# ccuchengwei/LongReadSelfCorrect

Measured on AMD Instinct MI355X. Metric: corrected Mbases/s (whole node), higher is better.
Workload: dtype int64

## Files before the change

longreadselfcorrect_amd/csrc/capi_core.cpp:

```cpp
#include <cmath>
#include <limits>

#include "capi_internal.h"

using namespace lrsc;

static thread_local std::string g_last_error;

int lrsc::fail(int status, const std::string& msg)
{
    g_last_error = msg;
    return status;
}
int lrsc::hip_fail(hipError_t e, const char* what)
{
    g_last_error = std::string(what) + ": " + hipGetErrorString(e);
    return LRSC_ERR_DEVICE;
}

extern "C" const char* lrsc_strerror(int status)
{
    switch(status) {
        case LRSC_OK: return "ok";
        case LRSC_ERR_IO: return "I/O error";
// ... 61 lines not shown
    (void)hipDeviceGetAttribute(&cus, hipDeviceAttributeMultiprocessorCount, ctx->device);
    return (uint32_t)cus * 4u * per_simd;
}

Tunables lrsc::read_tunables(const lrsc_ctx* ctx)
{
    const int kIntMax = std::numeric_limits<int>::max();
    Tunables t;
    t.wp_prep_bytes = env_bytes("LRSC_WP_PREP_MB", 24ull << 30, 20);
    t.wp_lane_bytes = env_bytes("LRSC_WP_LANE_MB", 32ull << 30, 20);
    t.wp_lanes = env_clamped("LRSC_WP_LANES", resident_waves(ctx, 2) * 64u, 64, kIntMax);
    t.wp_gen_quorum = env_clamped("LRSC_WP_GEN_QUORUM", 70, 0, 100);
    t.wp_gen_wait = env_clamped("LRSC_WP_GEN_WAIT", 6, 0, kIntMax);
    t.wp_wide_cap = env_clamped("LRSC_WP_WIDE_CAP", kNarrowLeaves, 1, (int)kNarrowLeaves);
    t.wp_wave = env_clamped("LRSC_WP_WAVE", 1, 0, 2);
    { const char* e = std::getenv("LRSC_WP_BEGIN_SORT"); t.wp_begin_sort = e && e[0] != '0'; }
    t.dp_chunk_bytes = env_bytes("LRSC_DP_CHUNK_MB", 16ull << 30, 20);
    t.dp_align_waves = env_clamped("LRSC_DP_ALIGN_WAVES", 0, 0, kIntMax);
    t.msa_force_global = std::getenv("LRSC_MSA_FORCE_GLOBAL") != nullptr;
    t.msa_lds_max = env_clamped("LRSC_MSA_LDS_MAX", 0, 1, kIntMax);
    { const char* e = std::getenv("LRSC_MSA_BATCH"); t.msa_batch = !(e && e[0] == '0'); }
    t.profile = std::getenv("LRSC_CORRECT_PROFILE") != nullptr;
    t.wp_dump = std::getenv("LRSC_WP_DUMP") != nullptr;
    t.dp_debug = std::getenv("LRSC_DP_DEBUG") != nullptr;
    return t;
}

int lrsc::check_offsets(const uint64_t* off, uint32_t n_reads)
{
    if(!off) return fail(LRSC_ERR_ARG, "null read offsets");
// ... 128 lines not shown
```

longreadselfcorrect_amd/csrc/capi_correct.cpp:

```cpp
#include "capi_internal.h"

using namespace lrsc;

struct lrsc::CorrectScratch {
    DevBuf<ReadPlan> d_plan;
    DevBuf<uint32_t> d_pieces;
    DevBuf<uint8_t> d_codes_out;
    DevBuf<uint64_t> d_dst_off;
    DevBuf<char> d_dst;
    DevBuf<double> d_freqs;
    DpStage stage;
    DevBuf<WpReadWork> d_work;
    DevBuf<WpRead> d_reads;
    DevBuf<WpSlot> d_slots;
    DevBuf<uint64_t> d_sz;
    DevBuf<uint32_t> d_key, d_key_tmp, d_list, d_list_tmp;
    DevBuf<uint32_t> d_small;
    DevBuf<WpDpItem> d_items, d_items2, d_items3;
    DevBuf<DevCounters> d_ctr2;
    hipEvent_t ev_side_t0 = nullptr, ev_side_t1 = nullptr;
    DevBuf<WpRequest> d_req;
    DevBuf<uint8_t> d_prep, d_lane, d_lane_side, d_lane_wide;
    DevBuf<uint32_t> d_wide_list;
    DevBuf<uint32_t> d_sort9;
// ... 165 lines not shown
    a.plan_stats = small(kWpSmallPlanStats); a.queue = small(kWpSmallQueue); a.n_dp_items = small(kWpSmallDpItems);
    a.n_req_out = small(kWpSmallReqOut);
    a.n_sort9 = small(kWpSmallSort9); a.begin_sort = tn.wp_begin_sort ? 1u : 0u;
    a.req_out = sc.d_req.p; a.req_cap = n;
    a.out_codes = sc.d_codes_out.p; a.piece_start = sc.d_pieces.p;
    a.auto_dp = (!p.no_dp && p.next_target == 1) ? 1u : 0u;
    a.general_quorum_pct = tn.wp_gen_quorum; a.general_max_wait = tn.wp_gen_wait;
    a.ctr = ctx->d_ctr;
    if(b->debug_flags & LRSC_DEBUG_WALKS) {
        if(!b->d_walk_log) HIP_TRY(hipMalloc(reinterpret_cast<void**>(&b->d_walk_log), b->seed_cap));
        HIP_TRY(hipMemsetAsync(b->d_walk_log, 0, b->seed_cap, ctx->stream));
        a.walk_log = b->d_walk_log;
        b->walk_log_done = false;
    }
    if(tn.profile) {
        HIP_TRY(sc.d_prof.reserve(36));
        HIP_TRY(hipMemsetAsync(sc.d_prof.p, 0, 36 * sizeof(unsigned long long), ctx->stream));
        a.prof = sc.d_prof.p;
        a.begin_stats = sc.d_prof.p + 32;
    }
    if(!sc.side) {
        int least = 0, greatest = 0;
        HIP_TRY(hipDeviceGetStreamPriorityRange(&least, &greatest));
        HIP_TRY(hipStreamCreateWithPriority(&sc.side, hipStreamNonBlocking, least));
    }
    if(!sc.ev_ready) HIP_TRY(hipEventCreateWithFlags(&sc.ev_ready, hipEventDisableTiming));
    return LRSC_OK;
}

void WpFlow::choose_range(uint32_t first)
{
    r0 = r1 = first;
// ... 127 lines not shown
    const WpLaneLayout LL = wp_lane_layout(lbytes, pathw);
    const uint64_t slots = tn.wp_lanes / 64;
    const uint64_t share = side ? wp_side_waves(tn) : slots;
    uint64_t lanes = std::min<uint64_t>(stride == 1 ? (((uint64_t)count + 63) & ~63ull) : count, share * 64 / stride);
    lanes = std::max<uint64_t>(1, std::min<uint64_t>(lanes, (tn.wp_lane_bytes / (side ? 4 : 1)) / LL.total));
    if(stride == 1) lanes = std::max<uint64_t>(64, lanes & ~63ull);
    DevBuf<uint8_t>& buf = side ? sc.d_lane_side : sc.d_lane;
    hipError_t e = buf.reserve(lanes * LL.total);
    if(e != hipSuccess) return e;
    x.list = list; x.reqs = rq; x.n_list = count;
    x.lane_ws = buf.p; x.lane_ws_bytes = LL.total; x.lane_pathw = pathw; x.n_lanes = (uint32_t)lanes; x.lane_stride = stride;
    x.queue = small(side ? kWpSmallSideQueue : kWpSmallExtQueue);
    e = hipMemsetAsync(x.queue, 0, sizeof(uint32_t), st);
    if(e != hipSuccess) return e;
    if(stride == 64 && tn.wp_wave != 0) return launch_wp_extend_wave(ctx->fm, x, st);
    return launch_wp_extend(ctx->fm, x, st);
}

int WpFlow::extension_launches(Round& R)
{
    return timed_launch(ctx, LRSC_K_EXTEND, [&]() -> hipError_t {
        hipError_t e = launch_wp_prepare(ctx->fm, a, ctx->stream);
        if(e == hipSuccess) e = launch_wp_begin(ctx->fm, a, ctx->stream);
        if(e != hipSuccess) return e;
        if(R.index != 0)
            return extend_range(a, a.list, a.reqs, R.n_ent, std::max(R.stats[2], 1u), ctx->stream, false,
                                R.n_ent <= 16384 ? 64u : R.n_ent <= 65536 ? 16u : 1u);
        e = extend_range(a, R.ext_list + R.n_mid, nullptr, R.n_ent - R.n_mid, std::min(R.stats[2], kWpPathwSmall), ctx->stream, false, 1);
        if(e != hipSuccess || R.n_mid == 0) return e;
        if(p.no_dp || escalate) return extend_range(a, R.ext_list, nullptr, R.n_mid, R.stats[2], ctx->stream, false, 64);
        R.long_launch = true;
        return e;
    });
}

int WpFlow::escalate_walks(const WpArgs& x0, uint32_t n_ent, uint32_t pathw)
{
    HIP_TRY(sc.d_wide_list.reserve(n_ent));
    uint32_t* d_count = small(kWpSmallWideCount);
    HIP_TRY(hipMemsetAsync(d_count, 0, sizeof(uint32_t), ctx->stream));
    hipError_t e = launch_wp_wide_collect(x0, sc.d_wide_list.p, d_count, ctx->stream);
    if(e != hipSuccess) return hip_fail(e, "wp_wide_collect");
    uint32_t n_wide = 0;
// ... 152 lines not shown
{
    std::fprintf(stderr, "[lrsc] wp reads [%u, %u) round %u: %u entries, %u DP requests (%llu strings), arenas q %.1f MB prep %.1f MB path %.1f MB, %llu walks escalated so far\n",
                 r0, r1, R.index, R.n_ent, R.n_items, (unsigned long long)sc.stage.n_strings, R.tot[0] / 1048576.0, R.tot[1] / 1048576.0, R.tot[2] / 1048576.0,
                 (unsigned long long)n_escalated);
    const unsigned long long* g = R.begin_stats;
    if(tn.wp_begin_sort)
        std::fprintf(stderr, "[lrsc] wp reads [%u, %u) round %u: wp_begin %llu interval lists, %llu entries, every list sorted (LRSC_WP_BEGIN_SORT)\n",
                     r0, r1, R.index, g[0], g[2] + g[3]);
    else
        std::fprintf(stderr, "[lrsc] wp reads [%u, %u) round %u: wp_begin %llu interval lists, %llu with a repeated code (%.1f%%); entries %llu in the lists without one, %llu in those with one\n",
                     r0, r1, R.index, g[0], g[1], 100.0 * g[1] / std::max(g[0], 1ull), g[2], g[3]);
}

int WpFlow::print_extension_profile()
{
    unsigned long long prs[32];
    HIP_TRY(hipStreamSynchronize(ctx->stream));
    HIP_TRY(hipStreamSynchronize(sc.side));
    HIP_TRY(hipMemcpy(prs, sc.d_prof.p, sizeof(prs), hipMemcpyDeviceToHost));
    for(int part = 0; part < 2; ++part) {
        const unsigned long long* pr = prs + 16 * part;
        if(pr[10] == 0) continue;
        const double all = (double)pr[10], st = (double)std::max<unsigned long long>(pr[11], 1);
        std::fprintf(stderr, "[lrsc] wp extension kernel (%s), lane wall ticks: %.3g total, %.0f per step over %.3g steps; extendLeaves %.1f%% (refine %.1f%%, attempToExtend %.1f%% of which "
                             "getFMIndexExtensions %.1f%%; SelectFreqsOfrange %.1f%%), PrunedBySeedSupport %.1f%%, materialise+commit %.1f%%, isTerminated %.1f%%, refill %.1f%%, finish %.1f%%; single-leaf fast steps %.1f%% of the steps in %.1f%% of the ticks\n",
                     part ? "long-gap walks, one per wavefront" : "bulk and later rounds",
                     all, all / st, st, 100 * pr[0] / all, 100 * pr[1] / all, 100 * pr[2] / all, 100 * pr[3] / all, 100 * pr[13] / all, 100 * pr[4] / all, 100 * pr[5] / all, 100 * pr[6] / all,
                     100 * pr[8] / all, 100 * pr[9] / all, 100 * pr[12] / st, 100 * pr[7] / all);
    }
    return LRSC_OK;
}

int WpFlow::gather_results(lrsc_read_result* res, uint64_t* piece_off, uint64_t piece_cap, char* out, uint64_t out_cap,
                           uint64_t* n_pieces_out, uint64_t* out_used)
{
    std::vector<WpRead> ro(n);
    COPY_TRY(ctx, ro.data(), sc.d_reads.p, (size_t)n * sizeof(WpRead), hipMemcpyDeviceToHost);
    std::vector<uint32_t> pieces(std::max<uint64_t>(piece_total, 1));
    if(piece_total) COPY_TRY(ctx, pieces.data(), sc.d_pieces.p, (size_t)piece_total * sizeof(uint32_t), hipMemcpyDeviceToHost);
    std::vector<uint64_t> dst_off(n + 1, 0);
    uint64_t n_pieces = 0;
    for(uint32_t r = 0; r < n; ++r) {
        const WpRead& o = ro[r];
// ... 81 lines not shown
```

longreadselfcorrect_amd/csrc/capi_internal.h:

```cpp
#pragma once
#include <hip/hip_runtime_api.h>

#include <algorithm>
#include <cstdint>
#include <cstdio>
#include <cstdlib>
#include <cstring>
#include <map>
#include <mutex>
#include <new>
#include <string>
#include <vector>

#include "../../include/lrsc.h"
#include "fm_layout.h"
#include "fm_locate.h"
#include "fm_pack.h"
#include "kernels.h"
#include "extend.h"
#include "correct_dev.h"
#include "dp_dev.h"
#include "wp.h"
#include "saipb.h"

// ... 43 lines not shown
            ++cur; off = 0;
        }
        auto* c = new(std::nothrow) DevBuf<uint8_t>();
        if(!c) return hipErrorOutOfMemory;
        hipError_t e = c->reserve(std::max<size_t>(bytes + bytes / 8, 64u << 20));
        if(e != hipSuccess) { delete c; return e; }
        chunks.push_back(c);
        cur = chunks.size() - 1;
        *out = c->p; off = bytes;
        return hipSuccess;
    }
};

struct Tunables {
    bool profile, wp_dump, dp_debug;
    uint32_t wp_wide_cap, wp_wave, wp_lanes;
    bool wp_begin_sort;
    uint64_t wp_prep_bytes, wp_lane_bytes;
    uint32_t wp_gen_quorum, wp_gen_wait;
    uint64_t dp_chunk_bytes;
    uint32_t dp_align_waves;
    bool msa_batch, msa_force_global;
    uint32_t msa_lds_max;
};

struct DeviceCopy {
    void* blocks[2] = {nullptr, nullptr};
    uint64_t* dollars[2] = {nullptr, nullptr};
    uint32_t* dollar_dir[2] = {nullptr, nullptr};
    void* ktab[5] = {nullptr, nullptr, nullptr, nullptr, nullptr};
    FmIndexDev dev{};
// ... 176 lines not shown
```

longreadselfcorrect_amd/csrc/walk_device.h:

```cpp
#pragma once
#include <hip/hip_runtime.h>

#include "extend.h"
#include "introsort_emul.h"
#include "rank_device.h"

#ifndef LRSC_WALK_NOINLINE
#define LRSC_WALK_NOINLINE __noinline__
#endif
#ifndef LRSC_WALK_FN
#define LRSC_WALK_FN __device__
#endif
#ifndef LRSC_WALK_TRACE
#define LRSC_WALK_TRACE(kind, a, b)
#endif

namespace lrsc {

constexpr uint64_t kNoKey = ~0ull;

template <bool WIDE>
LRSC_WALK_FN __forceinline__ void prepare_offset(const FmIndexDev& fm, const StrandC<typename Lay<WIDE>::pos_t>& sf,
                                               const StrandC<typename Lay<WIDE>::pos_t>& sr, const uint32_t* __restrict__ mtab,
                                               const uint8_t* __restrict__ q, uint32_t i, uint32_t Lq, uint32_t trg0,
// ... 502 lines not shown
#pragma unroll
            for(uint32_t j = 0; j < 4; ++j) e[j] = cur[i + j < n_cur ? i + j : i].localErr;
#pragma unroll
            for(uint32_t j = 0; j < 4; ++j) if(i + j < n_cur && e[j] < minimumErrorRate) minimumErrorRate = e[j];
        }
        uint32_t w = 0;
        for(uint32_t i = 0; i < n_cur; ++i) {
            const double errorRateDiff = cur[i].localErr - minimumErrorRate;
            if((errorRateDiff > 0.05 && currentLength > localK / 2) || (errorRateDiff > 0.1 && currentLength > 15)) {
                free_leaf_slots(cur[i]);
                continue;
            }
            if(w != i) leaf_move(&cur[w], &cur[i]);
            ++w;
        }
        n_cur = w;

        n_highfreq = 0;
        const int highfreqThreshold = PBcoverage > 60 ? (int)((uint64_t)(PBcoverage / 60) * 3) : 3;
        for(uint32_t i = 0; i < n_cur; ++i) {
            const Leaf<P> par = cur[i];
            Ext ext[4];
            uint32_t mask = 0;
            int count = 0;
            while(count < 2) {
                if(count == 1 && !(par.localErr == minimumErrorRate && n_cur > 1)) break;
                if(count == 1) { LRSC_WALK_TRACE(2, i, n_cur); }
                uint64_t tc;
                const uint64_t tg = tick();
                mask = getFMIndexExtensions_v(par.flo, par.fhi, par.rlo, par.rhi, par.tailLetterCount, par.suf_lo, ext, tc);
// ... 28 lines not shown
        ch.alive = 1;
        return ch;
    }

    LRSC_WALK_FN void extendLeaves()
    {
        n_nxt = 0;
        uint64_t t = tick();
        if(currentKmerSize > maxOverlap) refineSAInterval(cur, n_cur, maxOverlap);
        tock(1, t);
        t = tick();
        attempToExtend();
        tock(2, t);
        if(error) return;
        if(n_nxt == 0) {
            const uint64_t LowerBound = (currentKmerSize - 2) > minOverlap ? (currentKmerSize - 2) : minOverlap;
            const uint64_t ts = tick();
            const uint64_t ReduceSize = SelectFreqsOfrange(LowerBound, currentKmerSize, cur, n_cur);
            tock(8, ts);
            refineSAInterval(cur, n_cur, ReduceSize);
            attempToExtend();
            if(error) return;
            if(n_nxt == 0) {
                min_SA_threshold--;
                attempToExtend();
                min_SA_threshold++;
                if(error) return;
            }
        }
        if(n_nxt != 0) {
            currentLength++;
            currentKmerSize++;
            if(isInsufficientFreqs(n_highfreq, n_nxt)) {
                const uint64_t LowerBound = (currentKmerSize - 2) > minOverlap ? (currentKmerSize - 2) : minOverlap;
                const uint64_t ts = tick();
                const uint64_t ReduceSize = SelectFreqsOfrange(LowerBound, currentKmerSize, nxt, n_nxt);
                tock(8, ts);
                refineSAInterval(nxt, n_nxt, ReduceSize);
            }
        }
    }

    LRSC_WALK_FN LRSC_WALK_NOINLINE bool isSupportedByNewSeed(Leaf<P>& nd, uint64_t smallSeedIdx, uint64_t largeSeedIdx)
    {
        return seed_support_core(nd, smallSeedIdx, largeSeedIdx);
    }
    LRSC_WALK_FN __forceinline__ bool seed_support_core(Leaf<P>& nd, uint64_t smallSeedIdx, uint64_t largeSeedIdx)
    {
// ... 217 lines not shown
                else if(alive) { if(c < 64) alive_lo |= 1ull << c; else alive_hi |= 1ull << (c - 64); has_child |= 1u << parent[j]; }
            }
        }
    }

    LRSC_WALK_FN LRSC_WALK_NOINLINE void terminated_leaf(Leaf<P>& lf, const uint32_t* pw, uint32_t plen, int extra)
    {
        const int hit = term_scan(lf);
        if(hit < 0) return;
        if(lf.res_first == -1) {
            if(n_results >= max_results()) { error = LRSC_WALK_ERR_RESULTS; return; }
            ++n_results;
            lf.res_first = (int)n_results;
        }
        lf.res_second = hit;
        term_store(lf, hit, pw, plen, extra);
    }
    LRSC_WALK_FN __forceinline__ bool term_may_hit(uint64_t suf_lo) const
    {
        if(currentKmerSize >= minOverlap) {
            const uint32_t L = minOverlap < 16 ? (uint32_t)minOverlap : 16u;
            const uint32_t code = (uint32_t)(suf_lo & (L >= 16 ? 0xFFFFFFFFull : ((1ull << (2 * L)) - 1ull)));
            const uint32_t h = (code * 0x9E3779B1u) >> 25;
            if((((h < 64 ? tmask0 : tmask1) >> (h & 63u)) & 1ull) == 0) return false;
        }
        return true;
    }
    LRSC_WALK_FN __forceinline__ int term_scan(const Leaf<P>& lf) const
    {
        const bool fvalid = lf.flo <= lf.fhi, rvalid = lf.rlo <= lf.rhi;
// ... 248 lines not shown
            cyc_loop += __builtin_readcyclecounter() - t_step0;
        } else
            step_body();
        return true;
    }

    LRSC_WALK_FN void step_body()
    {
        {
            uint64_t t = tick();
            LRSC_WALK_TRACE(0, n_cur, 0);
            extendLeaves();
            tock(0, t);
            if(error) return;
            LRSC_WALK_TRACE(1, n_nxt, 0);
            t = tick();
            PrunedBySeedSupport();
            tock(4, t);
            t = tick();
            uint32_t survivors = (uint32_t)(__builtin_popcountll(alive_lo) + __builtin_popcountll(alive_hi));
            if constexpr(BIG) { survivors = 0; for(uint32_t w = 0; w < bits_words(n_nxt); ++w) survivors += (uint32_t)__builtin_popcountll(this->alive_bits[w]); }
            auto is_alive = [&](uint32_t c) -> bool {
                if constexpr(BIG) return bits_get(this->alive_bits, c);
                else return ((c < 64 ? alive_lo >> c : alive_hi >> (c - 64)) & 1ull) != 0;
            };
            ++steps;
            if(survivors > maxLeaves) {
                if(currentLength >= minLength)
                    for(uint32_t c = 0; c < n_nxt; ++c) {
                        if(!is_alive(c)) continue;
                        const Leaf<P>& par = cur[nxt[c].parent];
                        terminated_leaf(nxt[c], paths + (uint64_t)par.path * pathw, par.path_len, (int)nxt[c].ext);
                        if(error) return;
                    }
                n_cur = survivors;
                ended = true;
                return;
            }
            if constexpr(BIG) { for(uint32_t i = 0; i < n_cur; ++i) if(!bits_get(this->child_bits, i)) free_leaf_slots(cur[i]); }
            else for(uint32_t i = 0; i < n_cur; ++i) if(!((has_child >> i) & 1u)) free_leaf_slots(cur[i]);
            constexpr uint32_t G = kCommitGroup;
            uint32_t seen = 0, w = 0;
// ... 6 lines not shown
#pragma unroll
                for(uint32_t j = 0; j < G; ++j) { live[j] = c0 + j < n_nxt && is_alive(c0 + j); anylive = anylive || live[j]; }
                if(!anylive) continue;
#pragma unroll
                for(uint32_t j = 0; j < G; ++j) {
                    const Leaf<P>& lf = nxt[live[j] ? c0 + j : c0];
                    parent[j] = lf.parent; ring[j] = lf.ring; path[j] = lf.path; hist_size[j] = lf.hist_size; plen[j] = lf.path_len;
                    ext[j] = lf.ext; globalErr[j] = lf.globalErr;
                }
#pragma unroll
                for(uint32_t j = 0; j < G; ++j) {
                    if(!live[j]) continue;
                    bool further;
                    if constexpr(BIG) further = bits_get(this->seen_bits, parent[j]); else further = ((seen >> parent[j]) & 1u) != 0;
                    if(further) {
                        const uint32_t pr = ring[j], pp = path[j];
                        if constexpr(BIG) {
                            ring[j] = bits_take_lowest(this->ring_bits, this->cap);
                            path[j] = bits_take_lowest(this->path_bits, this->cap);
                        } else {
                            ring[j] = (uint32_t)__builtin_ctz(ring_free); ring_free &= ring_free - 1u;
                            path[j] = (uint32_t)__builtin_ctz(path_free); path_free &= path_free - 1u;
                        }
                        const uint32_t nlive = hist_size[j] - 1 < 100 ? hist_size[j] - 1 : 100;
                        const uint32_t nburst = (nlive * 8 + kCopyChunk16 * 16 - 1) / (kCopyChunk16 * 16);
                        burst_copy16(rings + (uint64_t)ring[j] * 100, rings + (uint64_t)pr * 100, nburst);
                        burst_copy4(paths + (uint64_t)path[j] * pathw, paths + (uint64_t)pp * pathw, (plen[j] + 16) >> 4);
                    }
                    if constexpr(BIG) bits_set(this->seen_bits, parent[j]); else seen |= 1u << parent[j];
                }
// ... 92 lines not shown
```

longreadselfcorrect_amd/csrc/wp.h:

```cpp
#pragma once
#include <hip/hip_runtime_api.h>
#include <stdint.h>

#include "correct_dev.h"
#include "dp_dev.h"
#include "extend.h"

namespace lrsc {

enum : uint32_t { kWpFmValid = 1u, kWpDpValid = 2u, kWpGeomBad = 4u };
enum : uint32_t { kWpReqFm = 0u, kWpReqDp = 1u };

struct alignas(16) WpSlot {
    uint32_t read, it;
    uint64_t src_lo, src_hi;
    uint8_t k, next, rtou, flags;
    uint8_t dp_k, max_front, pad1, pad2;
    uint64_t dp_src_lo, dp_src_hi;
    uint32_t lq, gap, trg_len, pathw;
    uint32_t dp_lq;
    int32_t dp_total_freq;
    uint8_t* q;
    uint8_t* dpq;
    uint8_t* prep;
// ... 125 lines not shown
    const uint8_t* dp_cons;
    uint32_t n_dp;
    uint8_t* out_codes;
    uint32_t* piece_start;
    WpRequest* req_out;
    uint32_t* n_req_out;
    uint32_t req_cap;
    uint8_t* walk_log;
    DevCounters* ctr;
    unsigned long long* prof;
    uint32_t escalate;
    uint32_t* sort9;
    uint32_t* n_sort9;
    uint32_t begin_sort;
    unsigned long long* begin_stats;
};

constexpr uint32_t kWpPathwSmall = 64, kWpPathwMid = 256;

enum WpSmall : uint32_t {
    kWpSmallPlanStats = 0,
    kWpSmallQueue = 4,
    kWpSmallDpItems = 5,
    kWpSmallReqOut = 6,
    kWpSmallSort9 = 7,
    kWpSmallExtQueue = 8,
    kWpSmallSideQueue = 9,
    kWpSmallSideDpItems = 12,
    kWpSmallWideQueue = 13,
    kWpSmallWideCount = 14,
    kWpSmallWords = 16
};

hipError_t launch_wp_bounds(const WpArgs& a, ReadPlan* plan, hipStream_t stream);
hipError_t launch_wp_plan(const WpArgs& a, hipStream_t stream);
hipError_t launch_wp_materialize(const WpArgs& a, hipStream_t stream);
hipError_t launch_wp_prepare(const FmIndexDev& fm, const WpArgs& a, hipStream_t stream);
hipError_t launch_wp_begin(const FmIndexDev& fm, const WpArgs& a, hipStream_t stream);
hipError_t launch_wp_extend(const FmIndexDev& fm, const WpArgs& a, hipStream_t stream);
hipError_t launch_wp_extend_wave(const FmIndexDev& fm, const WpArgs& a, hipStream_t stream);
hipError_t wp_extend_wave_static_lds(bool wide, uint32_t* bytes);
hipError_t launch_wp_wide_collect(const WpArgs& a, uint32_t* out, uint32_t* n_out, hipStream_t stream);
hipError_t launch_wp_extend_wide(const FmIndexDev& fm, const WpArgs& a, hipStream_t stream);
hipError_t launch_wp_dp_collect(const WpArgs& a, const WpDpItem* items, hipStream_t stream);
hipError_t launch_wp_stitch(const WpArgs& a, hipStream_t stream);
hipError_t launch_wp_gather(const WpArgs& a, const uint64_t* dst_off, char* dst, hipStream_t stream);
hipError_t wp_scan(uint64_t* v, uint64_t n, void** tmp, size_t* tmp_cap, hipStream_t stream);
hipError_t wp_sort_list(const uint32_t* keys, uint32_t* keys_tmp, uint32_t* list, uint32_t* list_tmp, uint32_t n, void** tmp, size_t* tmp_cap, hipStream_t stream);

}
```

longreadselfcorrect_amd/csrc/wp.hip:

```cpp
#define LRSC_WALK_FN __device__ __forceinline__
#define LRSC_WALK_NOINLINE
#include <hip/hip_runtime.h>
#include <hipcub/hipcub.hpp>

#include <algorithm>

#include "walk_device.h"
#include "wp.h"
#include "wp_walk.h"

namespace lrsc {

constexpr uint64_t kWpBeginSortBlocks = 32768;

#ifndef LRSC_WP_EXTEND_OCC
#define LRSC_WP_EXTEND_OCC 2
#endif

struct WpGeom {
    int k, interval, trg_len, T_start, T_len;
    bool rtou, bad;
    uint32_t lq, pathw;
};
__device__ __forceinline__ WpGeom wp_geometry(const WpArgs& a, int S_seedLen, int S_end, int S_endBest, bool S_isRepeat, const int32_t* T)
// ... 315 lines not shown
        if(!fast && !want_gen && W.can_fast()) { W.enter_fast(L, pw); fast = true; }
        int r = 2;
        if(fast) {
            const uint64_t tq = prof ? __builtin_readcyclecounter() : 0;
            r = W.step_fast(L, pw);
            if(r != 1) fast = false;
            if(prof) { pr[7] += __builtin_readcyclecounter() - tq; if(r == 1) ++n_fast; }
        }
        const uint32_t n_fast_now = (uint32_t)__builtin_popcountll(__ballot(r == 1));
        if(r == 2) {
            const uint32_t n_need = (uint32_t)__builtin_popcountll(__ballot(true));
            const uint32_t n_busy = n_need + n_fast_now;
            const bool waited = __ballot(gen_wait >= a.general_max_wait) != 0;
            if(n_need * 100u < n_busy * a.general_quorum_pct && !waited) { ++gen_wait; want_gen = true; continue; }
            gen_wait = 0; want_gen = false;
            r = W.step() ? 1 : 0;
        }
        if(r == 1) continue;
        in_walk = false;
        const uint64_t tf0 = prof ? __builtin_readcyclecounter() : 0;
        wp_walk_finish(W, a, si, steps0);
        if(prof) t_finish += __builtin_readcyclecounter() - tf0;
    }
    if(prof && lane_id < a.n_lanes) {
        for(int j = 0; j < 8; ++j) atomicAdd(&a.prof[j], (unsigned long long)pr[j]);
        atomicAdd(&a.prof[8], (unsigned long long)t_refill);
        atomicAdd(&a.prof[9], (unsigned long long)t_finish);
        atomicAdd(&a.prof[10], (unsigned long long)(__builtin_readcyclecounter() - t_loop0));
        atomicAdd(&a.prof[11], (unsigned long long)W.steps);
        atomicAdd(&a.prof[12], (unsigned long long)n_fast);
        atomicAdd(&a.prof[13], (unsigned long long)pr[8]);
// ... 327 lines not shown
```

longreadselfcorrect_amd/csrc/wp_walk.h:

```cpp
#pragma once

namespace lrsc {

__device__ __forceinline__ uint64_t lanes_below(uint32_t lane) { return (1ull << lane) - 1ull; }
__device__ __forceinline__ uint32_t popc64(uint64_t m) { return (uint32_t)__builtin_popcountll(m); }
__device__ __forceinline__ uint32_t first_u32(uint32_t v) { return (uint32_t)__builtin_amdgcn_readfirstlane((int)v); }
__device__ __forceinline__ uint64_t first_u64(uint64_t v) { return (uint64_t)first_u32((uint32_t)v) | ((uint64_t)first_u32((uint32_t)(v >> 32)) << 32); }
__device__ __forceinline__ double first_f64(double v) { return __longlong_as_double((long long)first_u64((uint64_t)__double_as_longlong(v))); }
__device__ __forceinline__ uint32_t lane_u32(uint32_t v, uint32_t l) { return (uint32_t)__builtin_amdgcn_readlane((int)v, (int)l); }
__device__ __forceinline__ double lane_f64(double v, uint32_t l)
{
    const uint64_t b = (uint64_t)__double_as_longlong(v);
    return __longlong_as_double((long long)((uint64_t)lane_u32((uint32_t)b, l) | ((uint64_t)lane_u32((uint32_t)(b >> 32), l) << 32)));
}
__device__ __forceinline__ uint32_t wave_sum(uint32_t v)
{
    for(int o = 32; o > 0; o >>= 1) v += (uint32_t)__shfl_xor((int)v, o, 64);
    return first_u32(v);
}
__device__ __forceinline__ int wave_max(int v)
{
    for(int o = 32; o > 0; o >>= 1) { const int w = __shfl_xor(v, o, 64); v = w > v ? w : v; }
    return (int)first_u32((uint32_t)v);
}
__device__ __forceinline__ double wave_min(double v)
{
    for(int o = 32; o > 0; o >>= 1) { const double w = __shfl_xor(v, o, 64); v = w < v ? w : v; }
    return first_f64(v);
}
__device__ __forceinline__ void wave_sync()
{
    __builtin_amdgcn_fence(__ATOMIC_RELEASE, "workgroup");
    __builtin_amdgcn_wave_barrier();
    __builtin_amdgcn_fence(__ATOMIC_ACQUIRE, "workgroup");
}

template <bool WIDE, bool BIG>
__device__ __forceinline__ void wp_bind_static(Walk<WIDE, BIG>& W, const WpArgs& a, const WpSlot& s)
{
    using P = typename Lay<WIDE>::pos_t;
    const WpPrepLayout L = wp_prep_layout(s.lq, s.trg_len, a.seed_size, a.min_overlap, a.psz);
    uint8_t* ws = s.prep;
    W.q = s.q;
    W.Lq = s.lq; W.initk = s.k; W.path_len = s.gap; W.trg_len = s.trg_len; W.dis = (int32_t)s.gap;
    W.it9f = reinterpret_cast<SortItem*>(ws + L.item9f);
    W.it9r = reinterpret_cast<SortItem*>(ws + L.item9r);
    W.next9f = reinterpret_cast<uint16_t*>(ws + L.next9f);
    W.next9r = reinterpret_cast<uint16_t*>(ws + L.next9r);
    W.head9f = reinterpret_cast<uint16_t*>(ws + L.head9);
// ... 126 lines not shown
```

Before: 157.9.

## Deal leaf extensions across wavefront lanes in bulk per-lane walk kernel

```diff
diff --git a/longreadselfcorrect_amd/csrc/capi_core.cpp b/longreadselfcorrect_amd/csrc/capi_core.cpp
--- a/longreadselfcorrect_amd/csrc/capi_core.cpp
+++ b/longreadselfcorrect_amd/csrc/capi_core.cpp
@@ -99,6 +99,7 @@
     t.wp_gen_wait = env_clamped("LRSC_WP_GEN_WAIT", 6, 0, kIntMax);
     t.wp_wide_cap = env_clamped("LRSC_WP_WIDE_CAP", kNarrowLeaves, 1, (int)kNarrowLeaves);
     t.wp_wave = env_clamped("LRSC_WP_WAVE", 1, 0, 2);
+    t.wp_deal = env_clamped("LRSC_WP_DEAL", 1, 0, 1);
     { const char* e = std::getenv("LRSC_WP_BEGIN_SORT"); t.wp_begin_sort = e && e[0] != '0'; }
     t.dp_chunk_bytes = env_bytes("LRSC_DP_CHUNK_MB", 16ull << 30, 20);
     t.dp_align_waves = env_clamped("LRSC_DP_ALIGN_WAVES", 0, 0, kIntMax);
diff --git a/longreadselfcorrect_amd/csrc/capi_correct.cpp b/longreadselfcorrect_amd/csrc/capi_correct.cpp
--- a/longreadselfcorrect_amd/csrc/capi_correct.cpp
+++ b/longreadselfcorrect_amd/csrc/capi_correct.cpp
@@ -203,8 +203,8 @@
         b->walk_log_done = false;
     }
     if(tn.profile) {
-        HIP_TRY(sc.d_prof.reserve(36));
-        HIP_TRY(hipMemsetAsync(sc.d_prof.p, 0, 36 * sizeof(unsigned long long), ctx->stream));
+        HIP_TRY(sc.d_prof.reserve(kWpProfWords));
+        HIP_TRY(hipMemsetAsync(sc.d_prof.p, 0, kWpProfWords * sizeof(unsigned long long), ctx->stream));
         a.prof = sc.d_prof.p;
         a.begin_stats = sc.d_prof.p + 32;
     }
@@ -362,6 +362,7 @@
     e = hipMemsetAsync(x.queue, 0, sizeof(uint32_t), st);
     if(e != hipSuccess) return e;
     if(stride == 64 && tn.wp_wave != 0) return launch_wp_extend_wave(ctx->fm, x, st);
+    if(stride == 1 && tn.wp_deal != 0) return launch_wp_extend_deal(ctx->fm, x, st);
     return launch_wp_extend(ctx->fm, x, st);
 }
 
@@ -374,7 +375,9 @@
         if(R.index != 0)
             return extend_range(a, a.list, a.reqs, R.n_ent, std::max(R.stats[2], 1u), ctx->stream, false,
                                 R.n_ent <= 16384 ? 64u : R.n_ent <= 65536 ? 16u : 1u);
-        e = extend_range(a, R.ext_list + R.n_mid, nullptr, R.n_ent - R.n_mid, std::min(R.stats[2], kWpPathwSmall), ctx->stream, false, 1);
+        WpArgs xb = a;
+        if(a.prof) xb.gen_stats = a.prof + 36;
+        e = extend_range(xb, R.ext_list + R.n_mid, nullptr, R.n_ent - R.n_mid, std::min(R.stats[2], kWpPathwSmall), ctx->stream, false, 1);
         if(e != hipSuccess || R.n_mid == 0) return e;
         if(p.no_dp || escalate) return extend_range(a, R.ext_list, nullptr, R.n_mid, R.stats[2], ctx->stream, false, 64);
         R.long_launch = true;
@@ -557,7 +560,7 @@
 
 int WpFlow::print_extension_profile()
 {
-    unsigned long long prs[32];
+    unsigned long long prs[kWpProfWords];
     HIP_TRY(hipStreamSynchronize(ctx->stream));
     HIP_TRY(hipStreamSynchronize(sc.side));
     HIP_TRY(hipMemcpy(prs, sc.d_prof.p, sizeof(prs), hipMemcpyDeviceToHost));
@@ -570,6 +573,16 @@
                      part ? "long-gap walks, one per wavefront" : "bulk and later rounds",
                      all, all / st, st, 100 * pr[0] / all, 100 * pr[1] / all, 100 * pr[2] / all, 100 * pr[3] / all, 100 * pr[13] / all, 100 * pr[4] / all, 100 * pr[5] / all, 100 * pr[6] / all,
                      100 * pr[8] / all, 100 * pr[9] / all, 100 * pr[12] / st, 100 * pr[7] / all);
+    }
+    const unsigned long long* g = prs + 36;
+    if(g[0]) {
+        const double s = (double)g[0];
+        std::fprintf(stderr, "[lrsc] wp bulk launches, general steps of a wavefront: %llu, %.1f lanes taking part; leaves per step %.1f in all, %.2f per lane, %.2f in the widest "
+                             "(widest x lanes / all = %.2f; %.2f passes of 64 lanes); children after extendLeaves %.1f in all, %.2f per lane, %.2f in the widest "
+                             "(%.2f; %.2f passes); counters %llu %llu %llu %llu %llu %llu %llu %llu %llu %llu\n",
+                     g[0], g[1] / s, g[2] / s, (double)g[2] / std::max(g[1], 1ull), g[3] / s, (double)g[6] / std::max(g[2], 1ull), g[8] / s,
+                     g[4] / s, (double)g[4] / std::max(g[1], 1ull), g[5] / s, (double)g[7] / std::max(g[4], 1ull), g[9] / s,
+                     g[0], g[1], g[2], g[3], g[4], g[5], g[6], g[7], g[8], g[9]);
     }
     return LRSC_OK;
 }
diff --git a/longreadselfcorrect_amd/csrc/capi_internal.h b/longreadselfcorrect_amd/csrc/capi_internal.h
--- a/longreadselfcorrect_amd/csrc/capi_internal.h
+++ b/longreadselfcorrect_amd/csrc/capi_internal.h
@@ -81,7 +81,7 @@
 
 struct Tunables {
     bool profile, wp_dump, dp_debug;
-    uint32_t wp_wide_cap, wp_wave, wp_lanes;
+    uint32_t wp_wide_cap, wp_wave, wp_deal, wp_lanes;
     bool wp_begin_sort;
     uint64_t wp_prep_bytes, wp_lane_bytes;
     uint32_t wp_gen_quorum, wp_gen_wait;
diff --git a/longreadselfcorrect_amd/csrc/walk_device.h b/longreadselfcorrect_amd/csrc/walk_device.h
--- a/longreadselfcorrect_amd/csrc/walk_device.h
+++ b/longreadselfcorrect_amd/csrc/walk_device.h
@@ -540,6 +540,7 @@
             if(w != i) leaf_move(&cur[w], &cur[i]);
             ++w;
         }
+        if(w != n_cur) { LRSC_WALK_TRACE(8, n_cur - w, w); }
         n_cur = w;
 
         n_highfreq = 0;
@@ -598,6 +599,7 @@
         tock(2, t);
         if(error) return;
         if(n_nxt == 0) {
+            LRSC_WALK_TRACE(5, n_cur, 0);
             const uint64_t LowerBound = (currentKmerSize - 2) > minOverlap ? (currentKmerSize - 2) : minOverlap;
             const uint64_t ts = tick();
             const uint64_t ReduceSize = SelectFreqsOfrange(LowerBound, currentKmerSize, cur, n_cur);
@@ -606,6 +608,7 @@
             attempToExtend();
             if(error) return;
             if(n_nxt == 0) {
+                LRSC_WALK_TRACE(6, n_cur, 0);
                 min_SA_threshold--;
                 attempToExtend();
                 min_SA_threshold++;
@@ -616,6 +619,7 @@
             currentLength++;
             currentKmerSize++;
             if(isInsufficientFreqs(n_highfreq, n_nxt)) {
+                LRSC_WALK_TRACE(7, n_nxt, 0);
                 const uint64_t LowerBound = (currentKmerSize - 2) > minOverlap ? (currentKmerSize - 2) : minOverlap;
                 const uint64_t ts = tick();
                 const uint64_t ReduceSize = SelectFreqsOfrange(LowerBound, currentKmerSize, nxt, n_nxt);
@@ -863,6 +867,7 @@
             lf.res_first = (int)n_results;
         }
         lf.res_second = hit;
+        LRSC_WALK_TRACE(11, lf.res_first, 0);
         term_store(lf, hit, pw, plen, extra);
     }
     LRSC_WALK_FN __forceinline__ bool term_may_hit(uint64_t suf_lo) const
@@ -1141,7 +1146,14 @@
             tock(0, t);
             if(error) return;
             LRSC_WALK_TRACE(1, n_nxt, 0);
-            t = tick();
+        }
+        step_after_extend();
+    }
+
+    LRSC_WALK_FN void step_after_extend()
+    {
+        {
+            uint64_t t = tick();
             PrunedBySeedSupport();
             tock(4, t);
             t = tick();
@@ -1153,6 +1165,7 @@
             };
             ++steps;
             if(survivors > maxLeaves) {
+                LRSC_WALK_TRACE(10, survivors, 0);
                 if(currentLength >= minLength)
                     for(uint32_t c = 0; c < n_nxt; ++c) {
                         if(!is_alive(c)) continue;
@@ -1189,6 +1202,7 @@
                     bool further;
                     if constexpr(BIG) further = bits_get(this->seen_bits, parent[j]); else further = ((seen >> parent[j]) & 1u) != 0;
                     if(further) {
+                        LRSC_WALK_TRACE(9, parent[j], 0);
                         const uint32_t pr = ring[j], pp = path[j];
                         if constexpr(BIG) {
                             ring[j] = bits_take_lowest(this->ring_bits, this->cap);
diff --git a/longreadselfcorrect_amd/csrc/wp.h b/longreadselfcorrect_amd/csrc/wp.h
--- a/longreadselfcorrect_amd/csrc/wp.h
+++ b/longreadselfcorrect_amd/csrc/wp.h
@@ -163,7 +163,9 @@
     uint32_t* n_sort9;
     uint32_t begin_sort;
     unsigned long long* begin_stats;
-};
+    unsigned long long* gen_stats;
+};
+constexpr uint32_t kWpProfWords = 46;
 
 constexpr uint32_t kWpPathwSmall = 64, kWpPathwMid = 256;
 
@@ -187,6 +189,7 @@
 hipError_t launch_wp_prepare(const FmIndexDev& fm, const WpArgs& a, hipStream_t stream);
 hipError_t launch_wp_begin(const FmIndexDev& fm, const WpArgs& a, hipStream_t stream);
 hipError_t launch_wp_extend(const FmIndexDev& fm, const WpArgs& a, hipStream_t stream);
+hipError_t launch_wp_extend_deal(const FmIndexDev& fm, const WpArgs& a, hipStream_t stream);
 hipError_t launch_wp_extend_wave(const FmIndexDev& fm, const WpArgs& a, hipStream_t stream);
 hipError_t wp_extend_wave_static_lds(bool wide, uint32_t* bytes);
 hipError_t launch_wp_wide_collect(const WpArgs& a, uint32_t* out, uint32_t* n_out, hipStream_t stream);
diff --git a/longreadselfcorrect_amd/csrc/wp.hip b/longreadselfcorrect_amd/csrc/wp.hip
--- a/longreadselfcorrect_amd/csrc/wp.hip
+++ b/longreadselfcorrect_amd/csrc/wp.hip
@@ -353,7 +353,9 @@
             const bool waited = __ballot(gen_wait >= a.general_max_wait) != 0;
             if(n_need * 100u < n_busy * a.general_quorum_pct && !waited) { ++gen_wait; want_gen = true; continue; }
             gen_wait = 0; want_gen = false;
+            const uint32_t n_cur0 = W.n_cur;
             r = W.step() ? 1 : 0;
+            if(a.gen_stats) wp_gen_count(a.gen_stats, r == 1, n_cur0, W.n_nxt);
         }
         if(r == 1) continue;
         in_walk = false;
diff --git a/longreadselfcorrect_amd/csrc/wp_deal.hip b/longreadselfcorrect_amd/csrc/wp_deal.hip
--- /dev/null
+++ b/longreadselfcorrect_amd/csrc/wp_deal.hip
@@ -0,0 +1,149 @@
+#define LRSC_WALK_FN __device__ __forceinline__
+#define LRSC_WALK_NOINLINE
+#include <hip/hip_runtime.h>
+
+#include "walk_device.h"
+#include "wp.h"
+#include "wp_walk.h"
+#include "wp_deal_step.h"
+
+namespace lrsc {
+
+#ifndef LRSC_WP_EXTEND_OCC
+#define LRSC_WP_EXTEND_OCC 2
+#endif
+
+namespace {
+
+struct DevLanes {
+    static __device__ __forceinline__ uint32_t shfl(uint32_t v, uint32_t l) { return (uint32_t)__shfl((int)v, (int)l, 64); }
+    static __device__ __forceinline__ uint32_t shfl_up(uint32_t v, uint32_t o) { return (uint32_t)__shfl_up((int)v, o, 64); }
+    static __device__ __forceinline__ uint32_t lane(uint32_t v, uint32_t l) { return lane_u32(v, l); }
+    static __device__ __forceinline__ uint64_t ballot(bool b) { return __ballot(b); }
+    static __device__ __forceinline__ void sync() { wave_sync(); }
+};
+
+}
+
+template <bool WIDE, bool PROF>
+__global__ __launch_bounds__(64, LRSC_WP_EXTEND_OCC) void wp_extend_deal_kernel(FmIndexDev fm, WpArgs a)
+{
+    using P = typename Lay<WIDE>::pos_t;
+    __shared__ __attribute__((aligned(16))) uint32_t mtab[MaskTabSize<WIDE>::value];
+    init_mask_table<WIDE>(mtab);
+    const uint32_t lane = threadIdx.x;
+    const uint32_t lane_id = blockIdx.x * 64 + lane;
+    bool done = lane_id >= a.n_lanes;
+    Walk<WIDE> W;
+    wp_walk_consts(W, fm, a, mtab);
+    const WpLaneLayout LL = wp_lane_layout(a.lbytes, a.lane_pathw);
+    uint8_t* lws = a.lane_ws + (uint64_t)(done ? 0u : lane_id) * a.lane_ws_bytes;
+    Leaf<P>* const leaf_base = reinterpret_cast<Leaf<P>*>(lws + LL.leaves);
+    W.rings = reinterpret_cast<double*>(lws + LL.rings);
+    W.results = reinterpret_cast<WalkResultRec*>(lws + LL.results);
+    W.paths = reinterpret_cast<uint32_t*>(lws + LL.paths);
+    W.pathw = a.lane_pathw;
+    W.rpaths = W.paths + (uint64_t)32 * a.lane_pathw;
+    W.cur = leaf_base; W.nxt = leaf_base + 32; W.leaf_small = leaf_base;
+    W.n_cur = 0; W.n_nxt = 0; W.n_highfreq = 0; W.ended = false;
+    W.currentLength = 0; W.currentKmerSize = 0; W.maxOverlap = 0; W.maxLength = 0; W.maxIndelSize = 0; W.min_SA_threshold = 0;
+    W.head5 = nullptr; W.next5 = nullptr; W.flags5 = nullptr;
+
+    bool in_walk = false;
+    uint32_t si = 0;
+    uint64_t steps0 = 0;
+    Leaf<P> L;
+    uint32_t pw = 0;
+    bool fast = false;
+    uint32_t gen_wait = 0;
+    bool want_gen = false;
+    uint64_t pr[9] = {0, 0, 0, 0, 0, 0, 0, 0, 0};
+    uint64_t t_refill = 0, t_finish = 0, n_fast = 0;
+    const bool prof = PROF && a.prof != nullptr;
+    if constexpr(PROF) { if(prof) W.prof = pr; }
+    const uint64_t t_loop0 = prof ? __builtin_readcyclecounter() : 0;
+    while(true) {
+        int r = 3;
+        if(!done) {
+            if(!in_walk) {
+                const uint64_t tr0 = prof ? __builtin_readcyclecounter() : 0;
+                const uint32_t i = atomicAdd(a.queue, 1u);
+                if(i >= a.n_list) done = true;
+                else if(!(a.reqs && a.reqs[i].kind != kWpReqFm)) {
+                    si = a.list ? a.list[i] : (uint32_t)a.slot_base + i;
+                    const WpSlot& s = a.slots[si];
+                    if(!(s.flags & kWpGeomBad)) {
+                        W.cur = leaf_base; W.nxt = leaf_base + 32; W.leaf_small = leaf_base;
+                        steps0 = W.steps;
+                        wp_walk_bind(W, a, s);
+                        in_walk = true;
+                        fast = false; want_gen = false; gen_wait = 0;
+                    }
+                }
+                if(prof) t_refill += __builtin_readcyclecounter() - tr0;
+            }
+            if(in_walk) {
+                if(!fast && !want_gen && W.can_fast()) { W.enter_fast(L, pw); fast = true; }
+                r = 2;
+                if(fast) {
+                    const uint64_t tq = prof ? __builtin_readcyclecounter() : 0;
+                    r = W.step_fast(L, pw);
+                    if(r != 1) fast = false;
+                    if(prof) { pr[7] += __builtin_readcyclecounter() - tq; if(r == 1) ++n_fast; }
+                }
+            }
+        }
+        const uint64_t need = __ballot(r == 2);
+        if(need) {
+            const uint32_t n_need = popc64(need);
+            const uint32_t n_busy = n_need + popc64(__ballot(r == 1));
+            const bool waited = __ballot(r == 2 && gen_wait >= a.general_max_wait) != 0;
+            if(n_need * 100u < n_busy * a.general_quorum_pct && !waited) {
+                if(r == 2) { ++gen_wait; want_gen = true; r = 1; }
+            } else {
+                const bool act = r == 2;
+                if(act) { gen_wait = 0; want_gen = false; }
+                const uint32_t n_cur0 = W.n_cur;
+                const bool took = deal_step<DevLanes>(W, act, lane);
+                if(act) r = took ? 1 : 0;
+                if constexpr(PROF) { if(a.gen_stats) wp_gen_count(a.gen_stats, took, n_cur0, W.n_nxt); }
+            }
+        }
+        if(r == 0) {
+            in_walk = false;
+            const uint64_t tf0 = prof ? __builtin_readcyclecounter() : 0;
+            wp_walk_finish(W, a, si, steps0);
+            W.n_cur = 0; W.n_nxt = 0;
+            if(prof) t_finish += __builtin_readcyclecounter() - tf0;
+        }
+        if(__ballot(!done) == 0) break;
+    }
+    if(prof && lane_id < a.n_lanes) {
+        for(int j = 0; j < 8; ++j) atomicAdd(&a.prof[j], (unsigned long long)pr[j]);
+        atomicAdd(&a.prof[8], (unsigned long long)t_refill);
+        atomicAdd(&a.prof[9], (unsigned long long)t_finish);
+        atomicAdd(&a.prof[10], (unsigned long long)(__builtin_readcyclecounter() - t_loop0));
+        atomicAdd(&a.prof[11], (unsigned long long)W.steps);
+        atomicAdd(&a.prof[12], (unsigned long long)n_fast);
+        atomicAdd(&a.prof[13], (unsigned long long)pr[8]);
+    }
+    flush_counters(a.ctr, W.n_rank, W.n_blk);
+}
+
+hipError_t launch_wp_extend_deal(const FmIndexDev& fm, const WpArgs& a, hipStream_t stream)
+{
+    if(a.n_list == 0 || a.n_lanes == 0) return hipSuccess;
+    if(a.lane_stride > 1) return hipErrorInvalidValue;
+    const unsigned nb = (unsigned)(((uint64_t)a.n_lanes + 63) / 64);
+    const bool prof = a.prof != nullptr || a.gen_stats != nullptr;
+    if(fm.wide) {
+        if(prof) hipLaunchKernelGGL((wp_extend_deal_kernel<true, true>), dim3(nb), dim3(64), 0, stream, fm, a);
+        else     hipLaunchKernelGGL((wp_extend_deal_kernel<true, false>), dim3(nb), dim3(64), 0, stream, fm, a);
+    } else {
+        if(prof) hipLaunchKernelGGL((wp_extend_deal_kernel<false, true>), dim3(nb), dim3(64), 0, stream, fm, a);
+        else     hipLaunchKernelGGL((wp_extend_deal_kernel<false, false>), dim3(nb), dim3(64), 0, stream, fm, a);
+    }
+    return hipGetLastError();
+}
+
+}
diff --git a/longreadselfcorrect_amd/csrc/wp_deal_step.h b/longreadselfcorrect_amd/csrc/wp_deal_step.h
--- /dev/null
+++ b/longreadselfcorrect_amd/csrc/wp_deal_step.h
@@ -0,0 +1,231 @@
+#pragma once
+
+#ifndef LRSC_DEAL_TRACE
+#define LRSC_DEAL_TRACE(kind, a, b, c)
+#endif
+
+namespace lrsc {
+
+template <class X> LRSC_WALK_FN uint64_t deal_shfl_u64(uint64_t v, uint32_t l)
+{
+    return (uint64_t)X::shfl((uint32_t)v, l) | ((uint64_t)X::shfl((uint32_t)(v >> 32), l) << 32);
+}
+template <class X, class T> LRSC_WALK_FN T* deal_shfl_ptr(T* p, uint32_t l) { return reinterpret_cast<T*>(deal_shfl_u64<X>(reinterpret_cast<uint64_t>(p), l)); }
+template <class X> LRSC_WALK_FN uint32_t deal_incl_sum(uint32_t v, uint32_t lane)
+{
+    for(uint32_t o = 1; o < 64; o <<= 1) { const uint32_t w = X::shfl_up(v, o); if(lane >= o) v += w; }
+    return v;
+}
+
+struct Deal {
+    uint32_t incl, excl, total;
+};
+template <class X> LRSC_WALK_FN Deal deal_make(uint32_t cnt, uint32_t lane)
+{
+    Deal d;
+    d.incl = deal_incl_sum<X>(cnt, lane);
+    d.excl = d.incl - cnt;
+    d.total = X::lane(d.incl, 63);
+    return d;
+}
+template <class X> LRSC_WALK_FN uint32_t deal_owner(const Deal& d, uint32_t t)
+{
+    uint32_t lo = 0;
+    for(uint32_t s = 32; s > 0; s >>= 1) {
+        const uint32_t v = X::shfl(d.incl, lo + s - 1);
+        if(v <= t) lo += s;
+    }
+    return lo;
+}
+
+template <class X, bool WIDE>
+LRSC_WALK_FN void deal_refine(Walk<WIDE>& W, bool on, Leaf<typename Lay<WIDE>::pos_t>* leaves, uint32_t n, uint64_t l, uint32_t lane)
+{
+    using P = typename Lay<WIDE>::pos_t;
+    const Deal d = deal_make<X>(on ? n : 0u, lane);
+    if(lane == 0) { LRSC_DEAL_TRACE(3, d.total, 0, 0); }
+    for(uint32_t base = 0; base < d.total; base += 64) {
+        const uint32_t t = base + lane;
+        const bool have = t < d.total;
+        const uint32_t o = deal_owner<X>(d, have ? t : d.total - 1);
+        const uint32_t i = (have ? t : d.total - 1) - X::shfl(d.excl, o);
+        Leaf<P>* const arr = deal_shfl_ptr<X>(leaves, o);
+        const uint32_t ol = X::shfl((uint32_t)l, o);
+        if(have) W.find_suffix(arr[i], ol);
+    }
+    if(on) W.currentKmerSize = l;
+    X::sync();
+}
+
+template <class X, bool WIDE>
+LRSC_WALK_FN void deal_attempt(Walk<WIDE>& W, bool on, uint32_t lane)
+{
+    using P = typename Lay<WIDE>::pos_t;
+    double minimumErrorRate = 1;
+    if(on) {
+        for(uint32_t i = 0; i < W.n_cur; i += 4) {
+            double e[4];
+#pragma unroll
+            for(uint32_t j = 0; j < 4; ++j) e[j] = W.cur[i + j < W.n_cur ? i + j : i].localErr;
+#pragma unroll
+            for(uint32_t j = 0; j < 4; ++j) if(i + j < W.n_cur && e[j] < minimumErrorRate) minimumErrorRate = e[j];
+        }
+        uint32_t w = 0;
+        for(uint32_t i = 0; i < W.n_cur; ++i) {
+            const double errorRateDiff = W.cur[i].localErr - minimumErrorRate;
+            if((errorRateDiff > 0.05 && W.currentLength > W.localK / 2) || (errorRateDiff > 0.1 && W.currentLength > 15)) {
+                W.free_leaf_slots(W.cur[i]);
+                continue;
+            }
+            if(w != i) leaf_move(&W.cur[w], &W.cur[i]);
+            ++w;
+        }
+        W.n_cur = w;
+        W.n_highfreq = 0;
+    }
+    X::sync();
+    const int highfreqThreshold = W.PBcoverage > 60 ? (int)((uint64_t)(W.PBcoverage / 60) * 3) : 3;
+    const uint32_t my_cap = W.nxt == W.leaf_small ? W.small_cap() : W.max_children();
+    bool overflow = false;
+    const Deal d = deal_make<X>(on ? W.n_cur : 0u, lane);
+    if(lane == 0) { LRSC_DEAL_TRACE(0, d.total, 0, 0); }
+    for(uint32_t base = 0; base < d.total; base += 64) {
+        const uint32_t t = base + lane;
+        const bool have = t < d.total;
+        const uint32_t tt = have ? t : d.total - 1;
+        const uint32_t o = deal_owner<X>(d, tt);
+        const uint32_t o_excl = X::shfl(d.excl, o);
+        const uint32_t i = tt - o_excl;
+        Leaf<P>* const o_cur = deal_shfl_ptr<X>(W.cur, o);
+        Leaf<P>* const o_nxt = deal_shfl_ptr<X>(W.nxt, o);
+        const uint32_t o_n = X::shfl(W.n_cur, o), o_cap = X::shfl(my_cap, o);
+        const uint32_t o_count = X::shfl(W.n_nxt, o);
+        const double o_min = __builtin_bit_cast(double, deal_shfl_u64<X>(__builtin_bit_cast(uint64_t, minimumErrorRate), o));
+        const uint64_t o_sa = deal_shfl_u64<X>(W.min_SA_threshold, o), o_len = deal_shfl_u64<X>(W.currentLength, o),
+                       o_indel = deal_shfl_u64<X>(W.maxIndelSize, o);
+        uint16_t* const o_head5 = deal_shfl_ptr<X>(W.head5, o);
+        uint16_t* const o_next5 = deal_shfl_ptr<X>(W.next5, o);
+        const uint8_t* const o_flags5 = deal_shfl_ptr<X>(W.flags5, o);
+        const uint64_t s_sa = W.min_SA_threshold, s_len = W.currentLength, s_indel = W.maxIndelSize;
+        uint16_t* const s_head5 = W.head5;
+        uint16_t* const s_next5 = W.next5;
+        const uint8_t* const s_flags5 = W.flags5;
+        W.min_SA_threshold = o_sa; W.currentLength = o_len; W.maxIndelSize = o_indel;
+        W.head5 = o_head5; W.next5 = o_next5; W.flags5 = o_flags5;
+        Leaf<P> par = {};
+        typename Walk<WIDE>::Ext ext[4];
+        uint32_t mask = 0;
+        if(have) {
+            LRSC_DEAL_TRACE(1, base, o_excl, o_count);
+            par = o_cur[i];
+            int count = 0;
+            while(count < 2) {
+                if(count == 1 && !(par.localErr == o_min && o_n > 1)) break;
+                uint64_t tc;
+                mask = W.getFMIndexExtensions_v(par.flo, par.fhi, par.rlo, par.rhi, par.tailLetterCount, par.suf_lo, ext, tc);
+                if(mask != 0) break;
+                W.min_SA_threshold--;
+                count++;
+            }
+        }
+        W.min_SA_threshold = s_sa; W.currentLength = s_len; W.maxIndelSize = s_indel;
+        W.head5 = s_head5; W.next5 = s_next5; W.flags5 = s_flags5;
+        uint32_t v = 0;
+#pragma unroll
+        for(uint32_t b = 0; b < 4; ++b)
+            if((mask >> b) & 1u) v += 1u + (ext[b].freq > highfreqThreshold ? 0x10000u : 0u);
+        const uint32_t v_incl = deal_incl_sum<X>(v, lane), v_excl = v_incl - v;
+        const uint32_t first = o_excl > base ? o_excl - base : 0u;
+        const uint32_t off = o_count + ((v_excl - X::shfl(v_excl, first)) & 0xFFFFu);
+        if(have) {
+            uint32_t k = off;
+#pragma unroll
+            for(uint32_t b = 0; b < 4; ++b) {
+                if(!((mask >> b) & 1u)) continue;
+                if(k >= o_cap) { overflow = true; break; }
+                o_nxt[k++] = W.make_child(par, i, b, ext[b]);
+            }
+        }
+        const uint32_t s0 = d.excl > base ? d.excl : base, s1 = d.incl < base + 64 ? d.incl : base + 64;
+        const bool mine = on && s0 < s1;
+        const uint32_t sum = X::shfl(v_incl, mine ? s1 - 1 - base : 0u) - X::shfl(v_excl, mine ? s0 - base : 0u);
+        const uint64_t ovf = X::ballot(overflow);
+        if(mine) {
+            LRSC_DEAL_TRACE(2, base, d.excl, sum);
+            W.n_nxt += sum & 0xFFFFu; W.n_highfreq += sum >> 16;
+        }
+        uint64_t m = ovf;
+        while(m) {
+            const uint32_t l = (uint32_t)__builtin_ctzll(m);
+            m &= m - 1ull;
+            const uint32_t bad_owner = X::lane(o, l);
+            if(lane == bad_owner) W.error = LRSC_WALK_ERR_CHILDREN;
+        }
+        overflow = false;
+    }
+    X::sync();
+}
+
+template <class X, bool WIDE>
+LRSC_WALK_FN bool deal_step(Walk<WIDE>& W, bool act, uint32_t lane)
+{
+    if(act && (W.ended || W.error || !(W.n_cur != 0 && W.n_cur <= W.maxLeaves && W.currentLength <= W.maxLength))) act = false;
+    const bool took = act;
+    if(act) {
+        W.leaf_steps += W.n_cur;
+        if(W.n_cur > W.max_front) W.max_front = W.n_cur;
+        W.n_nxt = 0;
+    }
+    X::sync();
+    const uint64_t t_ext = W.tick();
+    uint64_t t = t_ext;
+    deal_refine<X>(W, act && W.currentKmerSize > W.maxOverlap, W.cur, W.n_cur, W.maxOverlap, lane);
+    if(took) W.tock(1, t);
+    t = W.tick();
+    deal_attempt<X>(W, act, lane);
+    if(took) W.tock(2, t);
+    if(W.error) act = false;
+    const bool lvl1 = act && W.n_nxt == 0;
+    if(X::ballot(lvl1)) {
+        uint64_t ReduceSize = 0;
+        if(lvl1) {
+            const uint64_t LowerBound = (W.currentKmerSize - 2) > W.minOverlap ? (W.currentKmerSize - 2) : W.minOverlap;
+            const uint64_t ts = W.tick();
+            ReduceSize = W.SelectFreqsOfrange(LowerBound, W.currentKmerSize, W.cur, W.n_cur);
+            W.tock(8, ts);
+        }
+        X::sync();
+        deal_refine<X>(W, lvl1, W.cur, W.n_cur, ReduceSize, lane);
+        deal_attempt<X>(W, lvl1, lane);
+        if(W.error) act = false;
+        const bool lvl2 = lvl1 && act && W.n_nxt == 0;
+        if(X::ballot(lvl2)) {
+            if(lvl2) W.min_SA_threshold--;
+            deal_attempt<X>(W, lvl2, lane);
+            if(lvl2) W.min_SA_threshold++;
+            if(W.error) act = false;
+        }
+    }
+    bool relax = false;
+    uint64_t RelaxSize = 0;
+    if(act && W.n_nxt != 0) {
+        W.currentLength++;
+        W.currentKmerSize++;
+        if(W.isInsufficientFreqs(W.n_highfreq, W.n_nxt)) {
+            const uint64_t LowerBound = (W.currentKmerSize - 2) > W.minOverlap ? (W.currentKmerSize - 2) : W.minOverlap;
+            const uint64_t ts = W.tick();
+            RelaxSize = W.SelectFreqsOfrange(LowerBound, W.currentKmerSize, W.nxt, W.n_nxt);
+            W.tock(8, ts);
+            relax = true;
+        }
+    }
+    if(X::ballot(relax)) {
+        X::sync();
+        deal_refine<X>(W, relax, W.nxt, W.n_nxt, RelaxSize, lane);
+    }
+    if(took) W.tock(0, t_ext);
+    if(act) W.step_after_extend();
+    return took;
+}
+
+}
diff --git a/longreadselfcorrect_amd/csrc/wp_walk.h b/longreadselfcorrect_amd/csrc/wp_walk.h
--- a/longreadselfcorrect_amd/csrc/wp_walk.h
+++ b/longreadselfcorrect_amd/csrc/wp_walk.h
@@ -33,6 +33,33 @@
     __builtin_amdgcn_fence(__ATOMIC_RELEASE, "workgroup");
     __builtin_amdgcn_wave_barrier();
     __builtin_amdgcn_fence(__ATOMIC_ACQUIRE, "workgroup");
+}
+
+__device__ __forceinline__ void wp_gen_count(unsigned long long* g, bool took, uint32_t n_cur, uint32_t n_nxt)
+{
+    const uint64_t m = __ballot(took);
+    if(m == 0) return;
+    uint32_t sum[2], mx[2];
+    for(int k = 0; k < 2; ++k) {
+        const uint32_t v = k ? n_nxt : n_cur;
+        bool cand = took;
+        sum[k] = 0; mx[k] = 0;
+        for(int b = 15; b >= 0; --b) {
+            const bool bit = took && ((v >> b) & 1u);
+            sum[k] += (uint32_t)__builtin_popcountll(__ballot(bit)) << b;
+            if(__ballot(cand && bit)) { mx[k] |= 1u << b; cand = cand && bit; }
+        }
+    }
+    if(threadIdx.x == (uint32_t)__builtin_ctzll(m)) {
+        atomicAdd(&g[0], 1ull);
+        atomicAdd(&g[1], (unsigned long long)__builtin_popcountll(m));
+        atomicAdd(&g[2], (unsigned long long)sum[0]); atomicAdd(&g[3], (unsigned long long)mx[0]);
+        atomicAdd(&g[4], (unsigned long long)sum[1]); atomicAdd(&g[5], (unsigned long long)mx[1]);
+        atomicAdd(&g[6], (unsigned long long)mx[0] * (unsigned long long)__builtin_popcountll(m));
+        atomicAdd(&g[7], (unsigned long long)mx[1] * (unsigned long long)__builtin_popcountll(m));
+        atomicAdd(&g[8], (unsigned long long)((sum[0] + 63u) / 64u));
+        atomicAdd(&g[9], (unsigned long long)((sum[1] + 63u) / 64u));
+    }
 }
 
 template <bool WIDE, bool BIG>
```

New measurement: 167.5 (median of 6 runs). +6.1%, better.
